# jliu/graph-normalizing-flows

Measured on AMD Instinct MI355X. Metric: node-updates/sec (fwd+logdet) on community_medium batch, higher is better.
Workload: dtype f32; 1 GPU; config2: community_medium batch=64/GPU (64 graphs total), 8-step GRevNet fwd+logdet, D=64 L=256 K=5 avg_then_mlp eps=1 leaky_relu(0.2), sparse topology+self loops; nodes_total=2718, edges_total=32202, nodes_rank0=2718, edges_rank0=32202, weights=N(0,2/(fan_in+fan_out)), seed 99, last layer x0.25, parallelism=single GPU

## Files before the change

graph-normalizing-flows_amd/csrc/gnf_fused.hip:

```cpp
#include <cstring>
#include "gnf_common.h"

namespace gnf {

static constexpr int kFusedThreads = 512;
static constexpr int kLdsLimit = 160 * 1024;
static constexpr int kRowptrPad = 40;
static constexpr int kColCap = 2048;

static inline int pad16(int v) { return (v + 15) & ~15; }

int64_t packed_floats(const GnfMlp* m) {
    int64_t tot = 0;
    for (int j = 0; j < m->num_layers; ++j) {
        const int64_t ip = pad16(m->dims[j]), op = pad16(m->dims[j + 1]);
        tot += 2 * ip * op + op;
    }
    return tot;
}

__global__ __launch_bounds__(256) void k_pack_layer(const float* __restrict__ W,
                                                    const float* __restrict__ b, int I, int O, int Ip,
                                                    int Op, float* __restrict__ wout,
                                                    float* __restrict__ bout, float* __restrict__ wtout) {
    const int64_t nw = (int64_t)Ip * Op;
    const int64_t i = (int64_t)blockIdx.x * 256 + threadIdx.x;
    if (i < nw) {
        const int q = (int)(i & 3);
        const int lane = (int)((i >> 2) & 63);
        const int64_t blk = i >> 8;
        const int kgs = Ip >> 4;
        const int nts = Op >> 4;
        const int kg = (int)(blk / nts), nt = (int)(blk % nts);
        (void)kgs;
        const int k = 16 * kg + 4 * (lane >> 4) + q;
        const int c = 16 * nt + (lane & 15);
        wout[i] = (k < I && c < O) ? W[(int64_t)k * O + c] : 0.f;
        const int nts_t = Ip >> 4;
        const int kg_t = (int)(blk / nts_t), nt_t = (int)(blk % nts_t);
        const int ko = 16 * kg_t + 4 * (lane >> 4) + q;
        const int ci = 16 * nt_t + (lane & 15);
        wtout[i] = (ci < I && ko < O) ? W[(int64_t)ci * O + ko] : 0.f;
    } else if (i < nw + Op) {
        const int c = (int)(i - nw);
        bout[c] = c < O ? b[c] : 0.f;
    }
}

static int64_t packed_weight_floats(const GnfMlp* m) {
    int64_t tot = 0;
    for (int j = 0; j < m->num_layers; ++j) tot += (int64_t)pad16(m->dims[j]) * pad16(m->dims[j + 1]);
    return tot;
}

int launch_pack_mlp(const GnfMlp* m, float* packed, hipStream_t st) {
    int64_t woff = 0, boff = packed_weight_floats(m);
    int64_t toff = boff;
    for (int j = 0; j < m->num_layers; ++j) toff += pad16(m->dims[j + 1]);
    for (int j = 0; j < m->num_layers; ++j) {
        const int I = m->dims[j], O = m->dims[j + 1], Ip = pad16(I), Op = pad16(O);
        const int64_t tot = (int64_t)Ip * Op + Op;
        hipLaunchKernelGGL(k_pack_layer, dim3((unsigned)((tot + 255) / 256)), dim3(256), 0, st, m->W[j],
                           m->b[j], I, O, Ip, Op, packed + woff, packed + boff, packed + toff + woff);
        GNF_LAUNCH_CHECK("k_pack_layer");
        woff += (int64_t)Ip * Op;
        boff += Op;
    }
    return GNF_OK;
}


}
#include "gnf_fused_dev.h"
#include "gnf_attn_front_dev.h"
namespace gnf {

#ifdef GNF_TRACE
static constexpr int kTraceSlots = 32, kTraceCoupled = kTraceSlots - 2, kTraceEnd = kTraceSlots - 1;
__shared__ unsigned long long s_trace[kFusedThreads / 64][kTraceSlots];
static unsigned long long* g_trace_buf = nullptr;
static int g_trace_cap = 0, g_trace_next = 0;
extern "C" __attribute__((visibility("default"))) void gnf_trace_set_buffer(unsigned long long* buf, int cap) {
    g_trace_buf = buf, g_trace_cap = cap, g_trace_next = 0;
}
__device__ __forceinline__ void geo_stamp(int slot) {
    __builtin_amdgcn_sched_barrier(0);
    const unsigned long long t = __builtin_readcyclecounter();
    if ((threadIdx.x & 63) == 0) s_trace[threadIdx.x >> 6][slot] = t;
    __builtin_amdgcn_sched_barrier(0);
}
__device__ __forceinline__ void geo_stamp_after(int slot, float landed) {
    asm volatile("" ::"v"(landed));
    geo_stamp(slot);
}
#define GNF_STAMP(SLOT) geo_stamp(SLOT)
#define GNF_STAMP_AFTER(SLOT, V) geo_stamp_after(SLOT, V)
#else
#define GNF_STAMP(SLOT) ((void)0)
#define GNF_STAMP_AFTER(SLOT, V) ((void)0)
#endif

struct CoupleOwn {
    float xu = 0.f;
    float* dst = nullptr;
    double* part = nullptr;
    double* sq_part = nullptr;
    int inverse = 0;
};
template <int TM, bool STASH, bool FRONT, bool ROWLD, bool PLAIN, class Args, class FArgs, class RArgs>
__device__ __forceinline__ void couple_tile(const Args& a, const FArgs& fa, const RArgs& rla, const int H, const int LS, float* s_lds,
                                            const float* t_lds, float* xn_lds, const float* bn_lds, double* red, int tile, int row0,
                                            int tid, int wave, int lane, [[maybe_unused]] const CoupleOwn& own = CoupleOwn{}) {
    [[maybe_unused]] auto bn_part = [&]() -> double* {
        if constexpr (PLAIN) return nullptr; else return a.bn_part;
    };
    double local = 0.0, local2 = 0.0;
    for (int idx = tid; idx < TM * H; idx += kFusedThreads) {
        const int rl = idx / H, f = idx - rl * H;
        const int r = row0 + rl;
        if (bn_part()) xn_lds[rl * LS + f] = 0.f;
        bool live;
        if constexpr (PLAIN) live = own.dst != nullptr; else live = r < a.n_nodes;
        if (live) {
            float sv = s_lds[rl * LS + f], tv = t_lds[rl * LS + f];
            [[maybe_unused]] const int HPb = (H + 15) & ~15;
            if constexpr (!PLAIN) {
                if (a.residual) {
                    float xr = a.x_cond[(int64_t)r * a.ld + f];
                    if constexpr (FRONT) {
                        if (fa.bn_part) xr = xr * bn_lds[f] + bn_lds[HPb + f];
                    }
                    sv += xr;
                    tv += xr;
                }
            }
            float xv;
            if constexpr (PLAIN) xv = own.xu; else xv = a.x_upd_src[(int64_t)r * a.ld + f];
            if constexpr (FRONT) {
                if (a.bnu_const) xv = xv * bn_lds[2 * HPb + f] + bn_lds[3 * HPb + f];
                else if (a.bnu_inv[0]) xv = (xv - bn_lds[f]) / bn_lds[HPb + f] * bn_lds[2 * HPb + f] + bn_lds[3 * HPb + f];
            }
            int inverse;
            if constexpr (PLAIN) inverse = own.inverse; else inverse = a.inverse;
            const float xn = inverse ? (xv - tv) * expf(-sv) : xv * expf(sv) + tv;
            if constexpr (PLAIN) *own.dst = xn; else a.x_upd[(int64_t)r * a.ld + f] = xn;
            local += (double)sv;
            local2 += (double)xn * (double)xn;
            if constexpr (ROWLD) s_lds[rl * LS + f] = sv;
            if (bn_part()) xn_lds[rl * LS + f] = xn;
            if constexpr (STASH) {
                a.stash_st[0][(int64_t)r * H + f] = sv;
                a.stash_st[1][(int64_t)r * H + f] = tv;
            }
        }
    }
    if constexpr (PLAIN) GNF_STAMP(kTraceCoupled);
    for (int off = 32; off > 0; off >>= 1) local += __shfl_down(local, off, 64);
    if constexpr (PLAIN) {
        constexpr int NW = kFusedThreads / 64;
        const bool sq = own.sq_part != nullptr;
        if (sq)
// ... 319 lines not shown
        }
        if constexpr (STASH && NETS == 2) {
            if (j >= 1) {
#pragma unroll
                for (int q = 0; q < 2; ++q)
                    tile_dump<TM, kFusedThreads, true>(buf(q, pp), LS, a.stash_act[q][j], (int64_t)a.stash_ld, a.stash_w[j - 1], row0,
                                                       a.n_nodes, tid);
            }
        }
        pp ^= 1;
        __syncthreads();
    }

    if constexpr (STASH) {
        const int total_words = 2 * (a.K - 1) * (MT * 4) * a.stash_mld;
        unsigned long long* gm = a.stash_mask + (size_t)tile * total_words;
        for (int i = tid; i < total_words; i += kFusedThreads) gm[i] = fmask[i];
    }
    if (NETS == 1) {
        const float* o_lds = buf(0, pp);
        float* dst = a.st_out[net0];
        for (int idx = tid; idx < TM * H; idx += kFusedThreads) {
            const int rl = idx / H, f = idx - rl * H;
            const int r = row0 + rl;
            if (r < a.n_nodes)
                dst[(int64_t)r * H + f] = o_lds[rl * LS + f] + (a.residual ? a.x_cond[(int64_t)r * a.ld + f] : 0.f);
        }
    } else {
        couple_tile<TM, STASH, FRONT, ROWLD, false>(a, fa, rla, H, LS, buf(0, pp), buf(1, pp), buf(0, pp ^ 1), bn_lds, red, tile, row0, tid,
                                                    wave, lane);
    }
}


struct GeoArgs {
    const int32_t* rowptr;
    const int32_t* col;
    const float* x_cond;
    float* x_upd;
    const float* x_upd_src;
    float* cond_copy;
    double* partials;
    double* sq_partials;
    const float* wp[2];
    int64_t ld;
    int32_t n_nodes, n_tiles;
    float eps, alpha;
    int32_t mean, act, inverse;
#ifdef GNF_TRACE
    unsigned long long* trace;
#endif
};

template <class T>
__device__ __forceinline__ T hold_v(T v) {
    asm volatile("" : "+v"(v));
    return v;
}
template <class T>
__device__ __forceinline__ T* hold_v(T* p) {
    asm volatile("" : "+v"(p));
    return (T*)(__attribute__((address_space(1))) T*)p;
}

template <int IN0G, int LG, int K, int HG>
struct GeoLayout {
    static constexpr int kWpn = 4;
    static constexpr int kFragFloats = 64 * 4;
    static_assert(kFragFloats * sizeof(float) == 1024 && sizeof(f32x4) == 16, "GNF_LOAD_B addresses 1 KiB fragment blocks, 16 bytes per lane");
    static_assert(K >= 2 && IN0G >= 1 && IN0G == HG, "combine = agg: the layer-0 input is as wide as the half that is rewritten");
    static_assert(LG == 4 * kWpn, "a wave owns exactly four column tiles of a hidden layer: one mlp_chunk<1, 4> per layer");
    static_assert(HG <= kWpn && LG <= kThinStages, "the output layer is at most one thin chunk per wave");
    static constexpr int ipg(int j) { return j == 0 ? IN0G : LG; }
    static constexpr int ont(int j) { return j == K - 1 ? HG : LG; }
    static constexpr int woff(int j) { return j == 0 ? 0 : woff(j - 1) + ipg(j - 1) * ont(j - 1) * kFragFloats; }
    static constexpr int boff(int j) { return j == 0 ? 0 : boff(j - 1) + 16 * ont(j - 1); }
    static constexpr int kBias = woff(K);
    static constexpr int kLS = 16 * (LG > IN0G ? LG : IN0G) + 4;
    static constexpr int kRed = 2 * (kFusedThreads / 64);
    static constexpr size_t kLds = (size_t)2 * 2 * 16 * kLS * sizeof(float) + kRed * sizeof(double) + (kRowptrPad + kColCap) * sizeof(int);
    static_assert(woff(1) == 16 * IN0G * 16 * LG && kBias == 16 * IN0G * 16 * LG + (K - 2) * 256 * LG * LG + 16 * LG * 16 * HG,
                  "sum of Ip x Op over the layers");
    static_assert(kLds <= (size_t)kLdsLimit, "activation buffers in LDS");
};

template <int IN0G, int LG, int K, int HG>
__global__ __launch_bounds__(kFusedThreads) void k_half_fused_geo(const GeoArgs a) {
    extern __shared__ __attribute__((aligned(16))) float smem[];
    using G = GeoLayout<IN0G, LG, K, HG>;
    constexpr int TM = 16, WPN = G::kWpn, LS = G::kLS, H = 16 * HG, IN0 = 16 * IN0G;
    static_assert(TM * H == kFusedThreads && IN0 == H, "one own-row element per thread, the same one in the gather and in the coupling");
    GNF_STAMP(0);
    auto buf = [&](int net_, int pp_) -> float* { return smem + (2 * net_ + pp_) * TM * LS; };
    double* red = reinterpret_cast<double*>(smem + 2 * 2 * TM * LS);
    int* s_rowptr = reinterpret_cast<int*>(red + G::kRed);
    int* s_col = s_rowptr + kRowptrPad;

    const int tid = threadIdx.x;
    const int wave = __builtin_amdgcn_readfirstlane(tid >> 6), lane = tid & 63;
    const int nl = wave / WPN;
    const int wl = (wave % WPN + nl * (WPN / 2)) % WPN;
    const int voff = lane * 16;

    const float* wnet = a.wp[nl];
#ifdef GNF_TRACE
    asm volatile("" ::"s"(a.trace));
#endif
    asm volatile("" ::"s"(a.rowptr), "s"(a.col), "s"(a.x_cond), "s"(a.x_upd), "s"(a.x_upd_src), "s"(a.cond_copy), "s"(a.partials),
                 "s"(a.sq_partials), "s"(wnet), "s"(a.ld), "s"(a.n_nodes), "s"(a.n_tiles), "s"(a.eps), "s"(a.alpha), "s"(a.mean), "s"(a.act),
                 "s"(a.inverse));
    const int tile = nets2_tile(blockIdx.x, a.n_tiles);
    const int row0 = tile * TM;

    const int rp_row = row0 + (tid < TM ? tid : TM);
    const int rp_reg = a.rowptr[rp_row < a.n_nodes ? rp_row : a.n_nodes];
    CoupleOwn own;
    float xc_own;
    {
        const int r = row0 + tid / H, f = tid % H;
        const bool live = r < a.n_nodes;
        const int64_t at = (int64_t)(live ? r : a.n_nodes - 1) * a.ld + f;
        xc_own = a.x_cond[at];
        own.xu = a.x_upd_src[at];
        own.dst = hold_v(live ? a.x_upd + at : nullptr);
        own.part = hold_v(a.partials + tile);
        own.sq_part = hold_v(a.sq_partials ? a.sq_partials + tile : nullptr);
        own.inverse = hold_v(a.inverse);
    }
    __builtin_amdgcn_sched_barrier(0);

    auto chunk = [&](auto jc) -> WChunk {
        constexpr int j = decltype(jc)::value;
        WChunk c;
        c.wbase = wnet + G::woff(j);
        c.wbytes = (unsigned)G::ipg(j) * (unsigned)G::ont(j) * 1024u;
        c.ipg = G::ipg(j);
        c.ont = G::ont(j);
        c.boff = G::boff(j);
        c.nt0 = wl;
        c.nv = j == K - 1 ? 1 : 4;
        c.layer = j;
        return c;
    };
    const bool last_mine = wl < HG;

    if (tid <= TM) s_rowptr[tid] = rp_reg;
    __syncthreads();
    GNF_STAMP(1);

    const int seg_beg = s_rowptr[0];
    const int seg_len = s_rowptr[TM] - seg_beg;
    const bool staged = seg_len <= kColCap;
    int col_reg = 0;
    if (staged && tid < seg_len) col_reg = a.col[seg_beg + tid];
    __builtin_amdgcn_sched_barrier(0);
    f32x4 b_pre[kPF][4];
    prefetch_chunk(chunk(std::integral_constant<int, 0>{}), WPN, voff, b_pre, true);
    const float* bnet = wnet + G::kBias + 16 * wl + (lane & 15);
    BiasRegs<4> bias_h[K - 1];
#pragma unroll
    for (int j = 0; j < K - 1; ++j)
#pragma unroll
        for (int b = 0; b < 4; ++b) bias_h[j].v[b] = bnet[G::boff(j) + 16 * WPN * b];
    const BiasRegs<1> bias_o{{bnet[G::boff(K - 1) - (last_mine ? 0 : 16 * wl)]}};
    __builtin_amdgcn_sched_barrier(0);
    if (staged) {
        if (tid < seg_len) s_col[tid] = col_reg;
        for (int i = tid + kFusedThreads; i < seg_len; i += kFusedThreads) s_col[i] = a.col[seg_beg + i];
    }
    __syncthreads();
    GNF_STAMP(2);
    const TileAgg ta{a.col, a.x_cond, a.ld, a.n_nodes, row0, H, IN0, IN0, a.mean, 0, a.eps, a.cond_copy};
    tile_gather<TM, kFusedThreads, kColCap>(ta, s_rowptr, s_col, buf(0, 0), buf(1, 0), LS, nullptr, tid, OwnRow{xc_own});
    __syncthreads();
    GNF_STAMP(3);

    const float slope_h = a.act == GNF_ACT_RELU ? 0.f : a.alpha;
    epi_static_for<K>([&](auto jc) {
        constexpr int j = decltype(jc)::value;
        const float* in_lds = buf(nl, j & 1);
        float* out_lds = buf(nl, (j & 1) ^ 1);
        const WChunk c = chunk(jc);
        GNF_STAMP_AFTER(4 + 2 * j, b_pre[0][0][0]);
        if constexpr (j < K - 2) {
            mlp_chunk<1, 4>(in_lds, LS, c, chunk(std::integral_constant<int, j + 1>{}), WPN, bias_h[j], out_lds, slope_h, lane, b_pre, EpiArgs{}, true);
        } else if constexpr (j == K - 2) {
            const WChunk nx = last_mine ? chunk(std::integral_constant<int, K - 1>{}) : c;
            mlp_chunk<1, 4>(in_lds, LS, c, nx, WPN, bias_h[j], out_lds, slope_h, lane, b_pre, EpiArgs{}, true);
        } else {
            if (last_mine) mlp_chunk_thin(in_lds, LS, c, c, WPN, bias_o, out_lds, 1.f, lane, b_pre);
        }
        __syncthreads();
        GNF_STAMP(5 + 2 * j);
    });

    constexpr int pp = K & 1;
    couple_tile<TM, false, false, false, true>(a, 0, 0, H, LS, buf(0, pp), buf(1, pp), buf(0, pp ^ 1), nullptr, red, tile, row0, tid, wave, lane, own);
    GNF_STAMP(kTraceEnd);
#ifdef GNF_TRACE
    static_assert(4 + 2 * K <= kTraceCoupled, "stamp slots");
    if (a.trace && (blockIdx.x == 0 || blockIdx.x == gridDim.x / 2) && lane < kTraceSlots)
        a.trace[((blockIdx.x != 0) * (kFusedThreads / 64) + wave) * kTraceSlots + lane] = s_trace[wave][lane];
#endif
}

static int max_padded_width(const GnfMlp* m) {
    int w = 16;
    for (int j = 0; j <= m->num_layers; ++j) w = w > pad16(m->dims[j]) ? w : pad16(m->dims[j]);
    return w;
}

static int bias_total(const GnfMlp* m) {
    int t = 0;
    for (int j = 0; j < m->num_layers; ++j) t += pad16(m->dims[j + 1]);
    return t;
}

static size_t fused_lds_bytes(const GnfMlp* m, int MT, int NETS) {
    const int LS = max_padded_width(m) + 4;
    return (size_t)(2 * NETS * 16 * MT * LS + NETS * bias_total(m) + 2) * sizeof(float) + 8 * sizeof(double) +
           (GNF_MAX_LAYERS * 8 + kRowptrPad + kColCap) * sizeof(int);
}

bool fused_fits_lds(const GnfMlp* m) { return fused_lds_bytes(m, 1, 1) <= (size_t)kLdsLimit; }

static void choose_shape(const HalfStep& hs, int* mt, int* nets);
static int choose_big(const HalfStep& hs);

bool fused_supported(const HalfStep& hs) {
    const GnfMlp *s = hs.s_net, *t = hs.t_net;
    if (!s->packed || !t->packed) return false;
    if (s->num_layers != t->num_layers) return false;
    for (int j = 0; j <= s->num_layers; ++j)
        if (s->dims[j] != t->dims[j]) return false;
    return fused_lds_bytes(s, 1, 1) <= (size_t)kLdsLimit;
}

bool fused_supports_oop(const HalfStep& hs) {
    if (!fused_supported(hs) || hs.s_net->attn) return false;
    if (choose_big(hs)) return true;
    int mt, nets;
    choose_shape(hs, &mt, &nets);
    return nets == 2;
}

static void choose_shape(const HalfStep& hs, int* mt, int* nets) {
    const GnfMlp* s = hs.s_net;
    const int64_t tiles16 = (hs.n_nodes + 15) / 16;
    auto fits = [&](int m, int n) { return fused_lds_bytes(s, m, n) <= (size_t)kLdsLimit; };
    int m = 1, n = 1;
    const int64_t cus = big_cu_count();
    if (tiles16 > cus && fits(2, 2)) {
        m = 2, n = 2;
    } else if (fits(1, 2)) {
        m = 1, n = 2;
    } else if (tiles16 > cus && fits(2, 1)) {
        m = 2, n = 1;
    }
    if (const int64_t force = opt(OPT_FORCE_SHAPE)) {
        const int fm = (int)(force / 10), fn = (int)(force % 10);
        if ((fm == 1 || fm == 2) && (fn == 1 || fn == 2) && fits(fm, fn)) m = fm, n = fn;
    }
    if (s->attn && s->attn->layer_norm) n = 1;
    *mt = m;
    *nets = n;
}

static int choose_big(const HalfStep& hs) {
    const GnfMlp* s = hs.s_net;
    if (!big_supported(s, hs.H) || hs.mlp_stash) return 0;
    if (hs.n_nodes * hs.ld >= (int64_t(1) << 31)) return 0;
    if (s->attn && s->attn->layer_norm) return 0;
    if (const int64_t force = opt(OPT_FORCE_SHAPE)) {
        if (force == kForceBigLostPartner) return 4;
        return (force % 10 == 0 && force >= 10 && force <= 40) ? (int)(force / 10) : 0;
    }
    const int64_t g = (hs.n_nodes + 15) / 16, c = big_cu_count();
    if (g <= 2 * c) return 0;
    const double old_q = (double)((g + 2 * c - 1) / (2 * c));
    double big_q;
    if (g <= 8 * c) {
        big_q = 1.22 + 0.525 * (double)g / (double)(2 * c);
    } else {
// ... 26 lines not shown
    FrontArgs fa{};
    return MT == 1 && NETS == 2 && !choose_big(hs) && front_fold_ok(hs, &fa);
}

static size_t fused_front_lds_bytes(const GnfMlp* m, const FrontDims& d) {
    const int LS = max_padded_width(m) + 4;
    const size_t act = (size_t)2 * 2 * 16 * LS, fr = (size_t)front_lds(d).total;
    return ((act > fr ? act : fr) + 2 * (size_t)bias_total(m) + 2) * sizeof(float) + 8 * sizeof(double) + (GNF_MAX_LAYERS * 8) * sizeof(int) +
           (size_t)4 * d.Hp * sizeof(float);
}

static bool front_fold_ok(const HalfStep& hs, FrontArgs* fa) {
    const GnfMlp *s = hs.s_net, *t = hs.t_net;
    const GnfAttn *a0 = s->attn, *a1 = t->attn;
    if (!a0 || !a1) return false;
    if (!hs.attn_packed[0] || !hs.attn_packed[1]) return false;
    if (!(hs.n_edges > 0 && hs.n_edges < 24 * hs.n_nodes) || !attn_front_fused_ok(a0, hs.H)) return false;
    if (a1->num_heads != a0->num_heads || a1->kq_dim != a0->kq_dim || a1->v_dim != a0->v_dim || a1->out_dim != a0->out_dim ||
        a1->concat != a0->concat || a1->kq_dim_division != a0->kq_dim_division)
        return false;
    if (a0->layer_norm || opt(OPT_ATTN_KERNEL)) return false;
    const FrontDims d = front_dims(hs.H, a0->num_heads, a0->kq_dim, a0->v_dim, a0->out_dim);
    if (!((d.PW >> 4) <= 6 && (d.Hp >> 4) <= 2 && d.kq == 10 && d.vd == 10)) return false;
    const int in0 = s->dims[0];
    if ((d.C & 15) || (a0->concat && (hs.H & 15)) || (in0 & 15) || in0 != (a0->concat ? hs.H : 0) + d.C) return false;
    if (fused_front_lds_bytes(s, d) > (size_t)kLdsLimit) return false;
    if (hs.mlp_stash) {
        const MlpStashLayout SL = mlp_stash_layout(s, hs.n_nodes, hs.H);
        const size_t act_bytes = (size_t)2 * 2 * 16 * (max_padded_width(s) + 4) * sizeof(float);
        if (!attn_front_fixed_geometry(d) || act_bytes + (size_t)SL.mask_words * 8 > (size_t)front_lds(d).total * sizeof(float)) return false;
    }
    const AttnRegion R = attn_region(a0, hs.n_nodes, in0);
    float* const r = hs.attn_region;
    for (int q = 0; q < 2; ++q) {
        fa->packed[q] = hs.attn_packed[q];
        fa->qkv[q] = r ? r + R.qkv[q] : nullptr;
        fa->h0[q] = r ? r + R.h0[q] : nullptr;
        fa->agg_out[q] = r ? r + R.agg[q] : nullptr;
        fa->mz_out[q] = r ? r + R.stats[q] : nullptr;
    }
    fa->rowptr = hs.rowptr, fa->col = hs.col, fa->x = hs.x_cond, fa->ldx = hs.ld;
    fa->tiles = hs.attn_tiles;
    fa->n_nodes = (int32_t)hs.n_nodes;
    fa->concat = a0->concat ? 1 : 0;
    fa->in0 = in0;
    fa->d = d;
    fa->scale = a0->kq_dim_division ? 1.f / sqrtf((float)a0->kq_dim) : 1.f;
    return true;
}

MlpStashLayout mlp_stash_layout(const GnfMlp* net, int64_t n, int32_t H) {
    auto al = [](size_t v) { return (v + 63) / 64 * 64; };
    MlpStashLayout L;
    const int K = net->num_layers, lmax = hidden_max(net);
    L.ld_act = lmax;
    L.hidden = K > 1 ? K - 1 : 0;
    size_t off = 0;
    L.h0 = off, off += al((size_t)n * net->dims[0]);
    L.act_each = al((size_t)n * lmax);
    L.act = off, off += 2 * (size_t)L.hidden * L.act_each;
    L.st_each = al((size_t)n * H);
    L.st = off, off += 2 * L.st_each;
    L.mld = 1;
    for (int j = 1; j < K; ++j) L.mld = L.mld > pad16(net->dims[j]) / 16 ? L.mld : pad16(net->dims[j]) / 16;
    L.mask_words = 2 * L.hidden * 4 * L.mld;
    L.mask = off, off += al((size_t)((n + 15) / 16) * L.mask_words * 2);
    L.slot = off;
    return L;
}

bool fused_stash_shape(const GnfMlp* s, const GnfMlp* t, int64_t n) {
    if (!s->packed || !t->packed || s->num_layers != t->num_layers) return false;
    if (s->attn && s->attn->layer_norm) return false;
    for (int j = 0; j <= s->num_layers; ++j)
        if (s->dims[j] != t->dims[j]) return false;
    if (opt(OPT_FORCE_SHAPE)) return false;
    return (n + 15) / 16 <= big_cu_count() && fused_lds_bytes(s, 1, 2) <= (size_t)kLdsLimit;
}

template <int IN0G, int LG, int K, int HG>
static bool geo_matches(const HalfStep& hs, const FusedArgs& a) {
    using G = GeoLayout<IN0G, LG, K, HG>;
    const GnfMlp* s = hs.s_net;
    if (opt(OPT_FORCE_SHAPE) || s->attn || hs.mlp_stash || hs.row_logdet || a.bn_part || a.concat || a.h0[0]) return false;
    if (a.K != K || a.H != 16 * HG || a.in0 != 16 * IN0G || s->dims[K] != 16 * HG) return false;
    for (int j = 0; j < K; ++j) {
        if (s->dims[j] != 16 * G::ipg(j) || a.ipg[j] != G::ipg(j) || a.ont[j] != G::ont(j) || a.boff[j] != G::boff(j)) return false;
        if (a.wp[0][j] != a.wp[0][0] + G::woff(j) || a.wp[1][j] != a.wp[1][0] + G::woff(j)) return false;
    }
    return a.bias[0] == a.wp[0][0] + G::kBias && a.bias[1] == a.wp[1][0] + G::kBias && a.LS == G::kLS;
}

template <int IN0G, int LG, int K, int HG>
static int launch_geo(const FusedArgs& a, unsigned tiles, hipStream_t st) {
#ifdef GNF_TRACE
    constexpr int lds_limit = kLdsLimit - (int)sizeof(unsigned long long) * (kFusedThreads / 64) * kTraceSlots;
#else
    constexpr int lds_limit = kLdsLimit;
#endif
    GNF_ONCE_PER_DEVICE(GNF_HIP_TRY(hipFuncSetAttribute(reinterpret_cast<const void*>(k_half_fused_geo<IN0G, LG, K, HG>),
                                                        hipFuncAttributeMaxDynamicSharedMemorySize, lds_limit)));
    GeoArgs g{a.rowptr, a.col, a.x_cond, a.x_upd, a.x_upd_src, a.cond_copy, a.partials, a.sq_partials, {a.wp[0][0], a.wp[1][0]},
              a.ld, a.n_nodes, a.n_tiles, a.eps, a.alpha, a.mean, a.act, a.inverse};
#ifdef GNF_TRACE
    const size_t per_launch = (size_t)2 * (kFusedThreads / 64) * kTraceSlots;
    g.trace = g_trace_buf && g_trace_cap > 0 ? g_trace_buf + (size_t)(g_trace_next++ % g_trace_cap) * per_launch : nullptr;
#endif
    constexpr size_t lds = GeoLayout<IN0G, LG, K, HG>::kLds;
    hipLaunchKernelGGL((k_half_fused_geo<IN0G, LG, K, HG>), dim3(tiles), dim3(kFusedThreads), lds, st, g);
    GNF_LAUNCH_CHECK("k_half_fused_geo");
    return GNF_OK;
}

template <bool ROWLD>
static int launch_nets2(const FusedArgs& a, int MT, bool fold, const FrontArgs& fa, const RowLdArgs* rla, unsigned tiles, size_t lds,
                        size_t front_lds, hipStream_t st) {
    if (fold && attn_front_fixed_geometry(fa.d)) return launch_shape<1, 2, false, true, true, ROWLD>(a, tiles, front_lds, st, &fa, rla);
    if (fold) return launch_shape<1, 2, false, true, false, ROWLD>(a, tiles, front_lds, st, &fa, rla);
    return MT == 2 ? launch_shape<2, 2, false, false, false, ROWLD>(a, tiles, lds, st, nullptr, rla)
                   : launch_shape<1, 2, false, false, false, ROWLD>(a, tiles, lds, st, nullptr, rla);
}

int launch_half_fused(const HalfStep& hs, float* scratch, hipStream_t st) {
    const GnfMlp *s = hs.s_net, *t = hs.t_net;
    *hs.n_partials = 0;
    if (hs.n_nodes == 0) return GNF_OK;
    int MT, NETS;
    choose_shape(hs, &MT, &NETS);
    FusedArgs a{};
    a.rowptr = hs.rowptr;
    a.col = hs.col;
    a.x_cond = hs.x_cond;
    a.x_upd = hs.x_upd;
    a.x_upd_src = hs.x_upd_src ? hs.x_upd_src : hs.x_upd;
    a.cond_copy = hs.cond_copy;
    a.partials = hs.partials;
    a.sq_partials = NETS == 2 ? hs.sq_partials : nullptr;
    a.bn_part = NETS == 2 ? hs.bn_part : nullptr;
    a.st_out[0] = scratch;
    a.st_out[1] = scratch + hs.n_nodes * hs.H;
    FrontArgs fa{};
    const bool fold = s->attn && MT == 1 && NETS == 2 && !choose_big(hs) && front_fold_ok(hs, &fa);
    const bool rowld = hs.row_logdet != nullptr;
    const RowLdArgs rla{hs.row_logdet, hs.bnc_c};
    if (rowld && (hs.direction != GNF_FORWARD || hs.mlp_stash)) {
        set_error("internal: per-row log-det on an inverse half-step or beside the MLP-row stash");
        return GNF_EINVAL;
    }
    if (hs.bnu_inv) {
        if (!fold || hs.direction != GNF_INVERSE) {
            set_error("internal: batch norm on load (inverse) handed to a half-step that does not run the fused attention instance");
            return GNF_EINVAL;
        }
        a.bnu_inv[0] = hs.bnu_inv->gamma, a.bnu_inv[1] = hs.bnu_inv->beta;
        a.bnu_inv[2] = hs.bnu_inv->moving_mean, a.bnu_inv[3] = hs.bnu_inv->moving_variance;
        a.bnu_inv_eps = hs.bnu_inv->epsilon;
    }
    if (hs.bnc) {
        if (!fold || hs.direction != GNF_FORWARD) {
            set_error("internal: batch norm on load handed to a half-step that does not run the fused attention instance");
            return GNF_EINVAL;
        }
        fa.bn_part = hs.bnc_part, fa.bn_nparts = hs.bnc_nparts;
        fa.bn_gamma = hs.bnc->gamma, fa.bn_beta = hs.bnc->beta, fa.bn_eps = hs.bnc->epsilon;
        fa.bn_mean_out = hs.bnc->batch_mean, fa.bn_var_out = hs.bnc->batch_variance;
        fa.bn_logdet_out = hs.bnc_logdet, fa.bn_const_out = hs.bnc_const;
        a.bnu_const = hs.bnu_const;
    }
    if (s->attn) {
        if (!fold) {
            float* h0_pair[2];
            const int rc0 = launch_attn_pair(hs, scratch, h0_pair, st);
            if (rc0) return rc0;
            a.h0[0] = h0_pair[0];
            a.h0[1] = h0_pair[1];
        }
        a.residual = s->attn->residual ? 1 : 0;
    }
    int64_t off = 0;
    int boff = 0;
    for (int j = 0; j < s->num_layers; ++j) {
        const int ip = pad16(s->dims[j]), op = pad16(s->dims[j + 1]);
        a.wp[0][j] = s->packed + off;
        a.wp[1][j] = t->packed + off;
        a.ipg[j] = ip / 16;
        a.ont[j] = op / 16;
        a.boff[j] = boff;
        boff += op;
        off += (int64_t)ip * op;
    }
    a.bias[0] = s->packed + off;
    a.bias[1] = t->packed + off;
    a.bias_tot = boff;
    a.ld = hs.ld;
    a.n_nodes = (int32_t)hs.n_nodes;
    a.H = hs.H;
    a.in0 = s->dims[0];
    a.K = s->num_layers;
    a.LS = max_padded_width(s) + 4;
    a.mean = hs.gnn.agg == GNF_AGG_MEAN;
    a.concat = hs.gnn.combine == GNF_COMBINE_CONCAT;
    a.act = hs.gnn.activation;
    a.inverse = hs.direction == GNF_INVERSE;
    a.eps = hs.gnn.epsilon;
    a.alpha = hs.gnn.alpha;

    auto report = [&](int64_t wgs) {
        *hs.n_partials = (int32_t)wgs;
        if (hs.n_sq) *hs.n_sq = a.sq_partials ? (int32_t)wgs : 0;
        if (hs.n_bn) *hs.n_bn = a.bn_part ? (int32_t)wgs : 0;
        return GNF_OK;
    };
    int rc;
    if (const int big = choose_big(hs)) {
        a.sq_partials = hs.sq_partials;
        a.bn_part = nullptr;
        if (!s->attn) {
            rc = launch_aggregate(hs.rowptr, hs.col, hs.n_nodes, hs.x_cond, hs.ld, hs.H, a.mean, a.concat ? 1 : 0, a.eps, scratch,
                                  a.in0, st);
            if (rc) return rc;
            a.h0[0] = a.h0[1] = scratch;
            const HalfScratch hsl = half_scratch(hs.n_nodes, a.in0, hidden_max(s), hs.H);
            if (hs.split_epoch > 0 && big_cu_count() / 2 <= kBigSplitMax && hsl.split_fits()) {
                a.big_split_flag = reinterpret_cast<int*>(scratch + hsl.split_flags);
                a.big_split_s = scratch + hsl.split_s;
                a.big_epoch = hs.split_epoch;
                a.big_epoch_set = opt(OPT_FORCE_SHAPE) == kForceBigLostPartner ? -hs.split_epoch : hs.split_epoch;
            }
        }
        int n_wg = 0;
        rc = launch_half_big(a, hs.n_nodes, big, st, &n_wg, rowld ? hs.row_logdet : nullptr);
        return rc ? rc : report(n_wg);
    }
    const int64_t tiles = (hs.n_nodes + 16 * MT - 1) / (16 * MT);
    a.n_tiles = (int32_t)tiles;
    const size_t lds = fused_lds_bytes(s, MT, NETS);
    if (hs.mlp_stash && !(MT == 1 && NETS == 2)) {
        set_error("internal: MLP-row stash on a launch shape other than (1,2) (mlp_stash_supported is false there)");
        return GNF_EINVAL;
    }
    if (NETS == 2) {
        const size_t front_lds = fold ? fused_front_lds_bytes(s, fa.d) : 0;
        if (hs.mlp_stash) {
            const MlpStashLayout L = mlp_stash_layout(s, hs.n_nodes, hs.H);
            a.stash_h0 = hs.mlp_stash + L.h0;
            for (int q = 0; q < 2; ++q) {
                for (int j = 1; j < s->num_layers; ++j) a.stash_act[q][j] = hs.mlp_stash + L.act_of(q, j);
                a.stash_st[q] = hs.mlp_stash + L.st_of(q);
            }
            for (int j = 0; j < s->num_layers; ++j) a.stash_w[j] = s->dims[j + 1];
            a.stash_ld = L.ld_act;
            a.stash_mask = reinterpret_cast<unsigned long long*>(hs.mlp_stash + L.mask);
            a.stash_mld = L.mld;
            rc = fold ? launch_shape<1, 2, true, true, true>(a, (unsigned)tiles, front_lds, st, &fa)
                      : launch_shape<1, 2, true>(a, (unsigned)tiles, lds + (size_t)L.mask_words * sizeof(unsigned long long), st);
        } else if (MT == 1 && !fold && geo_matches<2, 16, 5, 2>(hs, a)) {
            rc = launch_geo<2, 16, 5, 2>(a, (unsigned)tiles, st);
        } else {
            rc = rowld ? launch_nets2<true>(a, MT, fold, fa, &rla, (unsigned)tiles, lds, front_lds, st)
                       : launch_nets2<false>(a, MT, fold, fa, nullptr, (unsigned)tiles, lds, front_lds, st);
        }
        return rc ? rc : report(tiles);
    }
    if (hs.x_upd_src || hs.cond_copy) {
        set_error("internal: out-of-place half-step on the one-net-per-workgroup shape (fused_supports_oop is false there)");
        return GNF_EINVAL;
    }
    const unsigned grid = (unsigned)(8 * ((tiles + 3) / 4));
    rc = MT == 2 ? launch_shape<2, 1>(a, grid, lds, st) : launch_shape<1, 1>(a, grid, lds, st);
    if (rc) return rc;
    if (s->attn && s->attn->layer_norm) {
        rc = launch_half_layer_norm(hs, a.st_out[0], a.st_out[1], nullptr, st);
        if (rc) return rc;
    }
    return launch_coupling(a.st_out[0], a.st_out[1], hs, nullptr, st);
}

}
```

graph-normalizing-flows_amd/csrc/gnf_fused_dev.h:

```cpp
#pragma once
#include <type_traits>
#include "gnf_common.h"

namespace gnf {

typedef float f32x4 __attribute__((ext_vector_type(4)));


static constexpr int kFusedPF = 2;

typedef unsigned int u32x4 __attribute__((ext_vector_type(4)));

struct FusedArgs {
    const int32_t* rowptr;
    const int32_t* col;
    const float* x_cond;
    float* x_upd;
    const float* x_upd_src;
    float* cond_copy;
    double* partials;
    double* sq_partials;
    double* bn_part;
    float* st_out[2];
    const float* h0[2];
// ... 208 lines not shown
        GNF_MFMA_STAGE(u)                                                                          \
        GNF_INTERLEAVE()                                                                           \
        __builtin_amdgcn_sched_barrier(0);                                                         \
    }
    int kg0 = 0;
    if (ipg >= R) {
        for (; kg0 + 2 * R <= ipg; kg0 += R) {
            GNF_ROUND(kg0)
        }
        prefetch_chunk(nx, ts, voff, b_pre, thin_ok);
        __builtin_amdgcn_sched_barrier(0);
        GNF_ROUND(kg0)
        kg0 += R;
    } else {
        prefetch_chunk(nx, ts, voff, b_pre, thin_ok);
        __builtin_amdgcn_sched_barrier(0);
    }
    const int rem = ipg - kg0;
#pragma unroll
    for (int u = 0; u < PF; ++u) {
        if (u < rem) {
            GNF_MFMA_STAGE(u)
        }
    }
#undef GNF_ROUND
#undef GNF_INTERLEAVE
#undef GNF_MFMA_STAGE
    [[maybe_unused]] int mlo = 0, mhi = 0;
    [[maybe_unused]] int my_word = 0;
    if constexpr (EPI == EPI_EX) {
        static_assert(MT * NV * 4 <= 64, "EPI_EX: one mask word per lane of the wave");
        const int e = lane < MT * NV * 4 ? lane : 0;
        const int em = e / (4 * NV), eb = (e >> 2) % NV, er = e & 3;
        my_word = (4 * em + er) * ea.mld + nt0 + ts * eb;
        if (ea.mode != 0) {
            unsigned long long w = ~0ull;
            if (ea.mask != nullptr && lane < MT * NV * 4) w = ea.mask[my_word];
            mlo = (int)(unsigned)w, mhi = (int)(unsigned)(w >> 32);
        }
    }
    if constexpr (EPI == EPI_PLAIN) {
#pragma unroll
        for (int m = 0; m < MT; ++m)
#pragma unroll
            for (int b = 0; b < NV; ++b)
#pragma unroll
                for (int r = 0; r < 4; ++r) {
                    const float v = acc[m][b][r];
                    const int rl = 16 * m + 4 * lgrp + r, col = 16 * (nt0 + ts * b) + lrow;
                    out_lds[rl * LS + col] = fmaxf(v, slope * v);
                }
    } else
    epi_static_for<MT * NV * 4>([&](auto e_c) {
                constexpr int e = decltype(e_c)::value;
                constexpr int m = e / (4 * NV), b = (e >> 2) % NV, r = e & 3;
                const float v = acc[m][b][r];
                const int rl = 16 * m + 4 * lgrp + r, col = 16 * (nt0 + ts * b) + lrow;
                {
                    float o;
                    if (ea.mode == 0) {
                        o = fmaxf(v, slope * v);
                        const unsigned long long bal = __ballot(o > 0.f);
                        asm volatile("s_nop 1\n\tv_writelane_b32 %0, %2, %4\n\tv_writelane_b32 %1, %3, %4"
                                     : "+v"(mlo), "+v"(mhi)
                                     : "s"((int)(unsigned)bal), "s"((int)(unsigned)(bal >> 32)), "n"(e));
                    } else {
                        const unsigned long long keep = ((unsigned long long)(unsigned)__builtin_amdgcn_readlane(mhi, e) << 32) |
                                                        (unsigned)__builtin_amdgcn_readlane(mlo, e);
                        const float vs = v * ea.act_slope;
                        asm volatile("s_nop 1\n\tv_cndmask_b32_e64 %0, %1, %2, %3" : "=v"(o) : "v"(vs), "v"(v), "s"(keep));
                    }
                    out_lds[rl * LS + col] = o;
                    if (ea.dump && ea.row0 + rl < ea.n_nodes && col < ea.width)
                        ea.dump[(int64_t)(ea.row0 + rl) * ea.dld + col] = o;
                }
            });
    if constexpr (EPI == EPI_EX) {
        if (ea.mode == 0 && ea.mask != nullptr && lane < MT * NV * 4)
            ea.mask[my_word] = ((unsigned long long)(unsigned)mhi << 32) | (unsigned)mlo;
    }
}



template <int TM, int NTHR, bool NT = false>
__device__ __forceinline__ void tile_dump(const float* __restrict__ src, int LS, float* __restrict__ dump, int64_t dld,
                                          int width, int row0, int n_nodes, int tid) {
    if (((width | (int)dld) & 3) == 0 && (reinterpret_cast<uintptr_t>(dump) & 15) == 0) {
        static_assert(NTHR % TM == 0, "whole threads per row");
        constexpr int TPR = NTHR / TM;
        const int w4 = width >> 2;
        const int rl = tid / TPR, c0 = tid - rl * TPR;
        const int r = row0 + rl;
        if (r < n_nodes) {
            const float* sp = src + rl * LS;
            float* dp = dump + (int64_t)r * dld;
            for (int c4 = c0; c4 < w4; c4 += TPR) {
                const f32x4 v = *reinterpret_cast<const f32x4*>(sp + 4 * c4);
                f32x4* d = reinterpret_cast<f32x4*>(dp + 4 * c4);
                if (NT)
                    __builtin_nontemporal_store(v, d);
                else
                    *d = v;
            }
        }
    } else {
        for (int i = tid; i < TM * width; i += NTHR) {
            const int rl = i / width, c = i - rl * width;
            const int r = row0 + rl;
            if (r < n_nodes) {
                if (NT)
                    __builtin_nontemporal_store(src[rl * LS + c], dump + (int64_t)r * dld + c);
                else
                    dump[(int64_t)r * dld + c] = src[rl * LS + c];
            }
        }
    }
}

struct TileAgg {
    const int32_t* col;
    const float* x_cond;
    int64_t ld;
    int n_nodes, row0, H, in0, in0p, mean, concat;
    float eps;
    float* cond_copy = nullptr;
};

struct NoOwnRow {};
struct OwnRow {
    float xc;
};

template <int TM, int NTHR, int COLCAP, class Own = NoOwnRow>
__device__ __forceinline__ void tile_gather(const TileAgg& t, const int* __restrict__ s_rowptr, const int* __restrict__ s_col,
                                            float* __restrict__ buf0, float* __restrict__ buf1, int LS,
                                            float* __restrict__ h0_out, int tid, const Own& own = Own{}) {
    const int seg_beg = s_rowptr[0];
    const int seg_len = s_rowptr[TM] - seg_beg;
    const bool staged = seg_len <= COLCAP;
    auto gather = [&](int beg, int end, const float* xf, auto colat) -> float {
        float s = 0.f;
        int e = beg;
        for (; e + 8 <= end; e += 8) {
            int ci[8];
            float vv[8];
#pragma unroll
            for (int q = 0; q < 8; ++q) ci[q] = colat(e + q);
#pragma unroll
            for (int q = 0; q < 8; ++q) vv[q] = xf[(int64_t)ci[q] * t.ld];
#pragma unroll
            for (int q = 0; q < 8; ++q) s += vv[q];
        }
        if (e < end) {
            int ci[7];
            float vv[7];
#pragma unroll
            for (int q = 0; q < 7; ++q) ci[q] = colat(e + q < end ? e + q : end - 1);
#pragma unroll
            for (int q = 0; q < 7; ++q) vv[q] = xf[(int64_t)ci[q] * t.ld];
#pragma unroll
            for (int q = 0; q < 7; ++q)
                if (e + q < end) s += vv[q];
        }
        return s;
    };
// ... 49 lines not shown
```

graph-normalizing-flows_amd/csrc/gnf_options.h:

```cpp
#pragma once
#include <atomic>
#include <stdint.h>

#include <hip/hip_runtime.h>

namespace gnf {

enum OptionId {
    OPT_FORCE_SHAPE = 0,
    OPT_ATTN_KERNEL,
    OPT_ATTN_BWD_ROWS,
    OPT_BWD_GENERIC,
    OPT_DW_GROUPED,
    OPT_DW_WIDE_UNITS,
    OPT_DW_THIN_ON_DW,
    OPT_COUNT
};

static constexpr int64_t kForceBigLostPartner = 49;
extern std::atomic<int64_t> g_options[OPT_COUNT];
inline int64_t opt(OptionId id) { return g_options[id].load(std::memory_order_relaxed); }

#define GNF_ONCE_PER_DEVICE(...)                                                     \
    do {                                                                               \
        static std::atomic<uint64_t> once_mask_{0};                                    \
        int once_dev_ = 0;                                                             \
        (void)hipGetDevice(&once_dev_);                                                \
        const uint64_t once_bit_ = 1ull << (once_dev_ & 63);                           \
        if (!(once_mask_.load(std::memory_order_acquire) & once_bit_)) {               \
            __VA_ARGS__;                                                               \
            once_mask_.fetch_or(once_bit_, std::memory_order_release);                 \
        }                                                                              \
    } while (0)

}
```

Measured before the change: 45.27 million node-updates/s.

## Interleave both coupling nets per wave in phased MFMA pipeline for geo kernel

Adds a PHASES variant of the fused geometric half-step kernel, now the default. In it every wave computes two column tiles of each hidden layer for both the s and t nets, alternating between them. Each phase prefetches the next phase's weights and activations into a register ring and flushes the previous net's activations behind a single barrier, so LDS writes and global weight loads overlap MFMA work. This is meant to replace per-layer full synchronisation and the idle waves of the old split where half the waves served each net. The cost is more register pressure and dense manual scheduling hints, with the old path still reachable through a force option.

```diff
diff --git a/graph-normalizing-flows_amd/csrc/gnf_fused.hip b/graph-normalizing-flows_amd/csrc/gnf_fused.hip
--- a/graph-normalizing-flows_amd/csrc/gnf_fused.hip
+++ b/graph-normalizing-flows_amd/csrc/gnf_fused.hip
@@ -77,6 +77,7 @@
 
 #ifdef GNF_TRACE
 static constexpr int kTraceSlots = 32, kTraceCoupled = kTraceSlots - 2, kTraceEnd = kTraceSlots - 1;
+static constexpr int kTracePhFlushed = 20;
 __shared__ unsigned long long s_trace[kFusedThreads / 64][kTraceSlots];
 static unsigned long long* g_trace_buf = nullptr;
 static int g_trace_cap = 0, g_trace_next = 0;
@@ -562,9 +563,11 @@
     static_assert(woff(1) == 16 * IN0G * 16 * LG && kBias == 16 * IN0G * 16 * LG + (K - 2) * 256 * LG * LG + 16 * LG * 16 * HG,
                   "sum of Ip x Op over the layers");
     static_assert(kLds <= (size_t)kLdsLimit, "activation buffers in LDS");
+    static_assert(LG == 2 * kPhaseTs && kPhaseTs == kFusedThreads / 64, "a wave owns exactly two column tiles of a hidden layer of EACH net: one mlp_phase per net and layer");
+    static_assert(2 * HG <= kWpn, "the output layer's 2 HG accumulator chains go to waves 0 .. 2 HG - 1: one per SIMD");
 };
 
-template <int IN0G, int LG, int K, int HG>
+template <int IN0G, int LG, int K, int HG, bool PHASES = false>
 __global__ __launch_bounds__(kFusedThreads) void k_half_fused_geo(const GeoArgs a) {
     extern __shared__ __attribute__((aligned(16))) float smem[];
     using G = GeoLayout<IN0G, LG, K, HG>;
@@ -582,7 +585,10 @@
     const int wl = (wave % WPN + nl * (WPN / 2)) % WPN;
     const int voff = lane * 16;
 
-    const float* wnet = a.wp[nl];
+    const float* wnet = a.wp[PHASES ? 0 : nl];
+    [[maybe_unused]] const float* wnet1 = a.wp[1];
+    [[maybe_unused]] const int wt_own = (wave + kPhaseTs - HG) % kPhaseTs;
+    if constexpr (PHASES) asm volatile("" ::"s"(wnet1));
 #ifdef GNF_TRACE
     asm volatile("" ::"s"(a.trace));
 #endif
@@ -635,14 +641,39 @@
     if (staged && tid < seg_len) col_reg = a.col[seg_beg + tid];
     __builtin_amdgcn_sched_barrier(0);
     f32x4 b_pre[kPF][4];
+    [[maybe_unused]] f32x4 ph_b_pre[kPhasePF][2];
+    [[maybe_unused]] auto ph_pf = [](int j) constexpr { return G::ipg(j) < kPhasePF ? G::ipg(j) : kPhasePF; };
+    [[maybe_unused]] f32x4 ph_bias[2][K - 1][2];
+    [[maybe_unused]] const int thin_net = wave >= HG && wave < 2 * HG;
+    [[maybe_unused]] const bool thin_mine = wave < 2 * HG;
+    [[maybe_unused]] const int thin_tile = thin_mine ? (thin_net ? wt_own : wave) : 0;
+    BiasRegs<4> bias_h[K - 1];
+    BiasRegs<1> bias_o;
+    if constexpr (PHASES) {
+        const __amdgpu_buffer_rsrc_t rs0 =
+            __builtin_amdgcn_make_buffer_rsrc(const_cast<float*>(wnet), 0, G::ipg(0) * G::ont(0) * 1024, 0x00020000);
+#pragma unroll
+        for (int u = 0; u < ph_pf(0); ++u)
+#pragma unroll
+            for (int b = 0; b < 2; ++b) ph_b_pre[u][b] = GNF_LOAD_B(rs0, voff, (u * G::ont(0) + wave + kPhaseTs * b) * 1024);
+#pragma unroll
+        for (int q = 0; q < 2; ++q) {
+            const float* bq = (q ? wnet1 : wnet) + G::kBias + 16 * (q ? wt_own : wave) + 4 * (lane >> 4);
+#pragma unroll
+            for (int j = 0; j < K - 1; ++j)
+#pragma unroll
+                for (int b = 0; b < 2; ++b) ph_bias[q][j][b] = *reinterpret_cast<const f32x4*>(bq + G::boff(j) + 16 * kPhaseTs * b);
+        }
+        bias_o.v[0] = (thin_net ? wnet1 : wnet)[G::kBias + G::boff(K - 1) + 16 * thin_tile + (lane & 15)];
+    } else {
     prefetch_chunk(chunk(std::integral_constant<int, 0>{}), WPN, voff, b_pre, true);
     const float* bnet = wnet + G::kBias + 16 * wl + (lane & 15);
-    BiasRegs<4> bias_h[K - 1];
 #pragma unroll
     for (int j = 0; j < K - 1; ++j)
 #pragma unroll
         for (int b = 0; b < 4; ++b) bias_h[j].v[b] = bnet[G::boff(j) + 16 * WPN * b];
-    const BiasRegs<1> bias_o{{bnet[G::boff(K - 1) - (last_mine ? 0 : 16 * wl)]}};
+    bias_o.v[0] = bnet[G::boff(K - 1) - (last_mine ? 0 : 16 * wl)];
+    }
     __builtin_amdgcn_sched_barrier(0);
     if (staged) {
         if (tid < seg_len) s_col[tid] = col_reg;
@@ -656,6 +687,42 @@
     GNF_STAMP(3);
 
     const float slope_h = a.act == GNF_ACT_RELU ? 0.f : a.alpha;
+    if constexpr (PHASES) {
+        const int lrow = lane & 15, lgrp = lane >> 4;
+        const int lane_at = lrow * LS + 4 * lgrp;
+        f32x4 acc_s[2], acc_t[2], a_pre[kPhasePF];
+#pragma unroll
+        for (int u = 0; u < ph_pf(0); ++u) a_pre[u] = *reinterpret_cast<const f32x4*>(buf(0, 0) + lane_at + 16 * u);
+        WChunk thin;
+        thin.wbase = (thin_net ? wnet1 : wnet) + G::woff(K - 1);
+        thin.wbytes = (unsigned)G::ipg(K - 1) * (unsigned)G::ont(K - 1) * 1024u;
+        thin.ipg = G::ipg(K - 1), thin.ont = G::ont(K - 1), thin.boff = G::boff(K - 1), thin.nt0 = thin_tile, thin.nv = 1, thin.layer = K - 1;
+        epi_static_for<K - 1>([&](auto jc) {
+            constexpr int j = decltype(jc)::value;
+            constexpr int pj = j & 1;
+#pragma unroll
+            for (int b = 0; b < 2; ++b) acc_s[b] = ph_bias[0][j][b];
+            GNF_STAMP(4 + 4 * j);
+            mlp_phase<G::ipg(j), G::ont(j), ph_pf(j), (j > 0), PH_NEXT_HIDDEN, G::ipg(j), G::ont(j), ph_pf(j)>(
+                buf(0, pj) + lane_at, wnet + G::woff(j), wave, acc_s, a_pre, ph_b_pre, acc_t, buf(1, pj) + lane_at + 16 * wt_own, slope_h,
+                buf(1, pj) + lane_at, wnet1 + G::woff(j), wt_own, thin, b_pre, voff, [&] { GNF_STAMP(5 + 4 * j); });
+#pragma unroll
+            for (int b = 0; b < 2; ++b) acc_t[b] = ph_bias[1][j][b];
+            GNF_STAMP(6 + 4 * j);
+            constexpr int jn = j + 1 < K - 1 ? j + 1 : j;
+            mlp_phase<G::ipg(j), G::ont(j), ph_pf(j), true, (j + 1 < K - 1 ? PH_NEXT_HIDDEN : PH_NEXT_THIN), G::ipg(jn), G::ont(jn), ph_pf(jn)>(
+                buf(1, pj) + lane_at, wnet1 + G::woff(j), wt_own, acc_t, a_pre, ph_b_pre, acc_s, buf(0, pj ^ 1) + lane_at + 16 * wave, slope_h,
+                buf(0, pj ^ 1) + lane_at, wnet + G::woff(jn), wave, thin, b_pre, voff, [&] { GNF_STAMP(7 + 4 * j); });
+        });
+        constexpr int po = (K - 1) & 1;
+        phase_flush(acc_t, buf(1, po) + lane_at + 16 * wt_own, slope_h);
+        GNF_STAMP(kTracePhFlushed);
+        phase_barrier();
+        GNF_STAMP(kTracePhFlushed + 1);
+        if (thin_mine) mlp_chunk_thin(buf(thin_net, po), LS, thin, thin, kPhaseTs, bias_o, buf(thin_net, po ^ 1), 1.f, lane, b_pre);
+        __syncthreads();
+        GNF_STAMP(kTracePhFlushed + 2);
+    } else
     epi_static_for<K>([&](auto jc) {
         constexpr int j = decltype(jc)::value;
         const float* in_lds = buf(nl, j & 1);
@@ -678,7 +745,7 @@
     couple_tile<TM, false, false, false, true>(a, 0, 0, H, LS, buf(0, pp), buf(1, pp), buf(0, pp ^ 1), nullptr, red, tile, row0, tid, wave, lane, own);
     GNF_STAMP(kTraceEnd);
 #ifdef GNF_TRACE
-    static_assert(4 + 2 * K <= kTraceCoupled, "stamp slots");
+    static_assert(4 + 2 * K <= kTraceCoupled && 4 + 4 * (K - 1) <= kTracePhFlushed, "stamp slots");
     if (a.trace && (blockIdx.x == 0 || blockIdx.x == gridDim.x / 2) && lane < kTraceSlots)
         a.trace[((blockIdx.x != 0) * (kFusedThreads / 64) + wave) * kTraceSlots + lane] = s_trace[wave][lane];
 #endif
@@ -871,7 +938,8 @@
 static bool geo_matches(const HalfStep& hs, const FusedArgs& a) {
     using G = GeoLayout<IN0G, LG, K, HG>;
     const GnfMlp* s = hs.s_net;
-    if (opt(OPT_FORCE_SHAPE) || s->attn || hs.mlp_stash || hs.row_logdet || a.bn_part || a.concat || a.h0[0]) return false;
+    const int64_t force = opt(OPT_FORCE_SHAPE);
+    if ((force && force != kForceGeoParent) || s->attn || hs.mlp_stash || hs.row_logdet || a.bn_part || a.concat || a.h0[0]) return false;
     if (a.K != K || a.H != 16 * HG || a.in0 != 16 * IN0G || s->dims[K] != 16 * HG) return false;
     for (int j = 0; j < K; ++j) {
         if (s->dims[j] != 16 * G::ipg(j) || a.ipg[j] != G::ipg(j) || a.ont[j] != G::ont(j) || a.boff[j] != G::boff(j)) return false;
@@ -880,14 +948,14 @@
     return a.bias[0] == a.wp[0][0] + G::kBias && a.bias[1] == a.wp[1][0] + G::kBias && a.LS == G::kLS;
 }
 
-template <int IN0G, int LG, int K, int HG>
+template <int IN0G, int LG, int K, int HG, bool PHASES>
 static int launch_geo(const FusedArgs& a, unsigned tiles, hipStream_t st) {
 #ifdef GNF_TRACE
     constexpr int lds_limit = kLdsLimit - (int)sizeof(unsigned long long) * (kFusedThreads / 64) * kTraceSlots;
 #else
     constexpr int lds_limit = kLdsLimit;
 #endif
-    GNF_ONCE_PER_DEVICE(GNF_HIP_TRY(hipFuncSetAttribute(reinterpret_cast<const void*>(k_half_fused_geo<IN0G, LG, K, HG>),
+    GNF_ONCE_PER_DEVICE(GNF_HIP_TRY(hipFuncSetAttribute(reinterpret_cast<const void*>(k_half_fused_geo<IN0G, LG, K, HG, PHASES>),
                                                         hipFuncAttributeMaxDynamicSharedMemorySize, lds_limit)));
     GeoArgs g{a.rowptr, a.col, a.x_cond, a.x_upd, a.x_upd_src, a.cond_copy, a.partials, a.sq_partials, {a.wp[0][0], a.wp[1][0]},
               a.ld, a.n_nodes, a.n_tiles, a.eps, a.alpha, a.mean, a.act, a.inverse};
@@ -896,7 +964,7 @@
     g.trace = g_trace_buf && g_trace_cap > 0 ? g_trace_buf + (size_t)(g_trace_next++ % g_trace_cap) * per_launch : nullptr;
 #endif
     constexpr size_t lds = GeoLayout<IN0G, LG, K, HG>::kLds;
-    hipLaunchKernelGGL((k_half_fused_geo<IN0G, LG, K, HG>), dim3(tiles), dim3(kFusedThreads), lds, st, g);
+    hipLaunchKernelGGL((k_half_fused_geo<IN0G, LG, K, HG, PHASES>), dim3(tiles), dim3(kFusedThreads), lds, st, g);
     GNF_LAUNCH_CHECK("k_half_fused_geo");
     return GNF_OK;
 }
@@ -1044,7 +1112,8 @@
             rc = fold ? launch_shape<1, 2, true, true, true>(a, (unsigned)tiles, front_lds, st, &fa)
                       : launch_shape<1, 2, true>(a, (unsigned)tiles, lds + (size_t)L.mask_words * sizeof(unsigned long long), st);
         } else if (MT == 1 && !fold && geo_matches<2, 16, 5, 2>(hs, a)) {
-            rc = launch_geo<2, 16, 5, 2>(a, (unsigned)tiles, st);
+            rc = opt(OPT_FORCE_SHAPE) == kForceGeoParent ? launch_geo<2, 16, 5, 2, false>(a, (unsigned)tiles, st)
+                                                         : launch_geo<2, 16, 5, 2, true>(a, (unsigned)tiles, st);
         } else {
             rc = rowld ? launch_nets2<true>(a, MT, fold, fa, &rla, (unsigned)tiles, lds, front_lds, st)
                        : launch_nets2<false>(a, MT, fold, fa, nullptr, (unsigned)tiles, lds, front_lds, st);
diff --git a/graph-normalizing-flows_amd/csrc/gnf_fused_dev.h b/graph-normalizing-flows_amd/csrc/gnf_fused_dev.h
--- a/graph-normalizing-flows_amd/csrc/gnf_fused_dev.h
+++ b/graph-normalizing-flows_amd/csrc/gnf_fused_dev.h
@@ -314,6 +314,129 @@
 }
 
 
+static constexpr int kPhaseTs = 8;
+static constexpr int kPhasePF = 2 * kPF, kPhaseR = kPhasePF + 1;
+enum { PH_NEXT_HIDDEN = 0, PH_NEXT_THIN = 1 };
+
+__device__ __forceinline__ void phase_barrier() {
+    __builtin_amdgcn_sched_barrier(0);
+    asm volatile("s_waitcnt lgkmcnt(0)\n\ts_barrier" ::: "memory");
+    __builtin_amdgcn_sched_barrier(0);
+}
+
+__device__ __forceinline__ void phase_flush(const f32x4 (&pend)[2], float* __restrict__ dst, float slope) {
+#pragma unroll
+    for (int b = 0; b < 2; ++b) {
+        f32x4 o;
+#pragma unroll
+        for (int r = 0; r < 4; ++r) {
+            const float v = pend[b][r];
+            o[r] = fmaxf(v, slope * v);
+        }
+        *reinterpret_cast<f32x4*>(dst + 16 * kPhaseTs * b) = o;
+    }
+}
+
+template <int IPG, int ONT, int PFI, bool FLUSH, int NXKIND, int NX_IPG, int NX_ONT, int PFO, class Behind>
+__device__ __forceinline__ void mlp_phase(const float* __restrict__ arow, const float* wbase, int nt0, f32x4 (&acc)[2],
+                                          f32x4 (&a_pre)[kPhasePF], f32x4 (&b_pre)[kPhasePF][2], const f32x4 (&pend)[2],
+                                          float* __restrict__ pend_dst, float slope, const float* __restrict__ nx_arow,
+                                          const float* nx_wbase, int nx_nt0, const WChunk& nx_thin, f32x4 (&b_thin)[kPF][4],
+                                          int voff, Behind&& behind_barrier) {
+    constexpr int R = kPhaseR;
+    static_assert(PFI <= IPG && PFI <= kPhasePF && PFO <= NX_IPG && PFO <= kPhasePF && IPG >= 2, "whole stages, inside the ring");
+    const __amdgpu_buffer_rsrc_t rsrc = __builtin_amdgcn_make_buffer_rsrc(const_cast<float*>(wbase), 0, IPG * ONT * 1024, 0x00020000);
+    const __amdgpu_buffer_rsrc_t nrsrc =
+        __builtin_amdgcn_make_buffer_rsrc(const_cast<float*>(nx_wbase), 0, NX_IPG * NX_ONT * 1024, 0x00020000);
+    const int wt[2] = {nt0 * 1024, (nt0 + kPhaseTs) * 1024};
+    const int nwt[2] = {nx_nt0 * 1024, (nx_nt0 + kPhaseTs) * 1024};
+    f32x4 a_ring[R], b_ring[R][2];
+#pragma unroll
+    for (int u = 0; u < PFI; ++u) {
+        a_ring[u] = a_pre[u];
+#pragma unroll
+        for (int b = 0; b < 2; ++b) b_ring[u][b] = b_pre[u][b];
+    }
+    constexpr int kFirstNxA = FLUSH ? 1 : 0;
+#pragma unroll
+    for (int kg = 0; kg < IPG; ++kg) {
+        if (kg + PFI < IPG) {
+            const int kn = kg + PFI;
+            a_ring[kn % R] = *reinterpret_cast<const f32x4*>(arow + 16 * kn);
+#pragma unroll
+            for (int b = 0; b < 2; ++b) b_ring[kn % R][b] = GNF_LOAD_B(rsrc, voff, wt[b] + kn * ONT * 1024);
+        }
+        if constexpr (NXKIND == PH_NEXT_HIDDEN) {
+#pragma unroll
+            for (int n = 0; n < PFO; ++n) {
+                const int at = PFO <= IPG ? IPG - PFO + n : n * IPG / PFO;
+                const int at_a = at > kFirstNxA ? at : kFirstNxA;
+                if (at == kg) {
+#pragma unroll
+                    for (int b = 0; b < 2; ++b) b_ring[(IPG + n) % R][b] = GNF_LOAD_B(nrsrc, voff, nwt[b] + n * NX_ONT * 1024);
+                }
+                if (at_a == kg) a_ring[(IPG + n) % R] = *reinterpret_cast<const f32x4*>(nx_arow + 16 * n);
+            }
+        } else {
+            if (kg == IPG - kPF) {
+                prefetch_chunk(nx_thin, kPhaseTs, voff, b_thin, true);
+                __builtin_amdgcn_sched_barrier(0);
+            }
+        }
+        if (FLUSH && kg == 0) phase_flush(pend, pend_dst, slope);
+#pragma unroll
+        for (int q = 0; q < 4; ++q)
+#pragma unroll
+            for (int b = 0; b < 2; ++b)
+                acc[b] = __builtin_amdgcn_mfma_f32_16x16x4f32(b_ring[kg % R][b][q], a_ring[kg % R][q], acc[b], 0, 0, 0);
+        if (FLUSH && kg == 0) {
+            __builtin_amdgcn_sched_group_barrier(0x008, 1, 0);
+            __builtin_amdgcn_sched_group_barrier(0x100, 1, 0);
+            __builtin_amdgcn_sched_group_barrier(0x002, 12, 0);
+            __builtin_amdgcn_sched_group_barrier(0x008, 1, 0);
+            __builtin_amdgcn_sched_group_barrier(0x200, 1, 0);
+            __builtin_amdgcn_sched_group_barrier(0x002, 12, 0);
+            __builtin_amdgcn_sched_group_barrier(0x008, 1, 0);
+            __builtin_amdgcn_sched_group_barrier(0x200, 1, 0);
+            __builtin_amdgcn_sched_group_barrier(0x008, 1, 0);
+            __builtin_amdgcn_sched_group_barrier(0x020, 1, 0);
+            __builtin_amdgcn_sched_group_barrier(0x008, 1, 0);
+            __builtin_amdgcn_sched_group_barrier(0x008, 1, 0);
+            __builtin_amdgcn_sched_group_barrier(0x020, 1, 0);
+            __builtin_amdgcn_sched_group_barrier(0x008, 1, 0);
+            __builtin_amdgcn_sched_group_barrier(0x008, 1, 0);
+            __builtin_amdgcn_sched_group_barrier(0x020, 2, 0);
+        } else {
+            __builtin_amdgcn_sched_group_barrier(0x008, 1, 0);
+            __builtin_amdgcn_sched_group_barrier(0x100, kPhasePF, 0);
+            __builtin_amdgcn_sched_group_barrier(0x008, 1, 0);
+            __builtin_amdgcn_sched_group_barrier(0x020, 1, 0);
+            __builtin_amdgcn_sched_group_barrier(0x008, 1, 0);
+            __builtin_amdgcn_sched_group_barrier(0x008, 1, 0);
+            __builtin_amdgcn_sched_group_barrier(0x020, 1, 0);
+            __builtin_amdgcn_sched_group_barrier(0x008, 1, 0);
+            __builtin_amdgcn_sched_group_barrier(0x008, 1, 0);
+            __builtin_amdgcn_sched_group_barrier(0x020, 1, 0);
+            __builtin_amdgcn_sched_group_barrier(0x008, 1, 0);
+            __builtin_amdgcn_sched_group_barrier(0x008, 1, 0);
+            __builtin_amdgcn_sched_group_barrier(0x020, 1, 0);
+        }
+        __builtin_amdgcn_sched_barrier(0);
+        if (FLUSH && kg == 0) {
+            phase_barrier();
+            behind_barrier();
+        }
+    }
+    if constexpr (NXKIND == PH_NEXT_HIDDEN) {
+#pragma unroll
+        for (int n = 0; n < PFO; ++n) {
+            a_pre[n] = a_ring[(IPG + n) % R];
+#pragma unroll
+            for (int b = 0; b < 2; ++b) b_pre[n][b] = b_ring[(IPG + n) % R][b];
+        }
+    }
+}
+
 
 template <int TM, int NTHR, bool NT = false>
 __device__ __forceinline__ void tile_dump(const float* __restrict__ src, int LS, float* __restrict__ dump, int64_t dld,
diff --git a/graph-normalizing-flows_amd/csrc/gnf_options.h b/graph-normalizing-flows_amd/csrc/gnf_options.h
--- a/graph-normalizing-flows_amd/csrc/gnf_options.h
+++ b/graph-normalizing-flows_amd/csrc/gnf_options.h
@@ -18,6 +18,7 @@
 };
 
 static constexpr int64_t kForceBigLostPartner = 49;
+static constexpr int64_t kForceGeoParent = 13;
 extern std::atomic<int64_t> g_options[OPT_COUNT];
 inline int64_t opt(OptionId id) { return g_options[id].load(std::memory_order_relaxed); }
 
```

After: 45.94 million node-updates/s, median of 6. 1.01x the previous value.
